# ansonb/FeTA_TMLR

Measured on AMD Instinct MI355X. Metric: graphs/sec fwd+bwd, ZINC batch (N<=37,d=64,K=16), higher is better.
Workload: dtype f32; 1 GPU; ZINC-shaped synthetic padded-graph batch, ChebConvDynamic block (attention + coefficient generator + spectral filter), fwd+bwd; graphs_per_gpu=128, global_batch=128, n_pad=37, d_model=64, heads=4, filter_order=4, k_eig=16, filter_mode=spectral, layers=3, norm=batch(per-rank stats), hip_graph=True, backward=single, two_phase=False, graph_collectives=False, ranks=1, parallelism=dp1

## Files before the change

### feta_tmlr_amd/csrc/block_bwd.hip

```cpp
#include <cstdlib>
#include <type_traits>

#include "feta_abi_common.h"
#include "feta_colsum.h"
#include "feta_ln.h"
#include "feta_lp.h"
#include "feta_rowops.h"

namespace feta {

typedef feta_attn_block_grad BwdArgs;

constexpr int kBbD = 64, kBbH = 4, kBbDH = 16;
constexpr int kBbP = kBbD + 4;
constexpr int kBbThreads = 512;
constexpr int kBbMaxGrid = 256;

template <class T>
__host__ __device__ inline int block_bwd_lds_bytes(int nt, bool gbn, bool gln = false, int heads = kBbH) {
  const int nr = 16 * nt, P = kBbD + Lp<T>::PAD;
  return (int)sizeof(T) * 7 * nr * P
         + 4 * (nr * (nr + 1)
                + heads * nr * 2 + nr
                + 8 * kBbD + 8 * 2 * 16
                + (gbn ? 5 * kBbD + reduce_scratch_floats(kBbD, 512) : 0)
                + (gln ? 8 * 2 * kBbD : 0));
}

#ifdef FETA_TIMING
__device__ unsigned long long feta_bbwd_stamps[4 * 8 * 8];
__device__ unsigned int feta_bbwd_launch;
#endif
#define BB_STAMP(i) FETA_RT_STAMP(feta_bbwd_stamps, feta_bbwd_launch, i)

__device__ __forceinline__ void acc_to(float* p, float v, bool first) {
  if (first) *p = v;
  else atomicAdd(p, v);
}

template <class T, int NT, bool SPLIT, bool LOOP, bool TWO>
__global__ __launch_bounds__(kBbThreads) void attn_block_bwd_kernel(BwdArgs a, ColsumPlan sums, int main_grid) {
  if ((int)blockIdx.x >= main_grid) {
    colsum_role<kBbThreads>(sums, (int)blockIdx.x - main_grid);
    return;
  }
  typedef Lp<T> L;
  typedef typename L::Op Op;
  typedef typename L::Vec Vec;
  constexpr int NS = TWO ? 2 : 1;
  constexpr int D = kBbD, DH = kBbDH, H = kBbH * NS, P = kBbD + L::PAD, NR = 16 * NT, PEP = NR + 1;
  constexpr int VEC = L::VEC, RV = D / VEC;
  const int tid = threadIdx.x, lane = tid & 63, wv = tid >> 6, lq = lane & 15, g = lane >> 4;
  const int hp = SPLIT ? ((int)blockIdx.x >= a.B ? 1 : 0) : 0;
  const int h = SPLIT ? 2 * hp + (wv & 1) : (wv & 3);
  const int role = SPLIT ? ((wv >> 1) & 1) : (wv >> 2);
  const int half = wv >> 2;
  const int ct = SPLIT ? 2 * hp + (wv & 1) : (wv & 3);
  const int ktile = wv & 3;
  auto mine_dc = [&](int rt) { return SPLIT ? rt == (wv >> 1) : (rt & 1) == (wv >> 2); };
  auto mine_dx = [&](int rt) { return (rt & 1) == (wv >> 2); };
  T* Qs = reinterpret_cast<T*>(lds_bytes());
  T* Ks = Qs + NR * P;
  T* Vs = Ks + NR * P;
  T* Ds = Vs + NR * P;
  T* Os = Ds + NR * P;
  T* Gt = Os + NR * P;
  T* X0 = Gt + NR * P;
  float* PE = reinterpret_cast<float*>(X0 + NR * P);
  float* ST = PE + NR * PEP;
  float* RS = ST + H * NR * 2;
  float* DBO = RS + NR;
  float* DBS = DBO + 8 * D;
  float* gv = DBS + 8 * 2 * 16;
  const T* gdy = reinterpret_cast<const T*>(a.dy);
  const T* gy1 = reinterpret_cast<const T*>(a.y1);
  const T* gqkv = reinterpret_cast<const T*>(a.qkv);
  const T* gout = reinterpret_cast<const T*>(a.out);
  const T* gd2 = reinterpret_cast<const T*>(a.dout2);
  const T* gpe = reinterpret_cast<const T*>(a.pe);
  const T* gx0 = reinterpret_cast<const T*>(a.x0);
  const bool gbn = a.bn1 != nullptr;
  const bool gln = a.ln1_gamma != nullptr, x0ln = a.x0_ln_gamma != nullptr;
  const bool has_y1 = a.y1 != nullptr;
  float* DGL = gv;
  const bool has_pe = a.pe != nullptr;
  const bool want_sums = a.sum_out != nullptr;
  const bool xbn = a.bn0 != nullptr;
  const bool d2_f32 = a.dout2 != nullptr && a.dout2_f32 != 0 && sizeof(T) != sizeof(float);
  BB_STAMP(0);

  if (gbn) {
    float* scr = gv + 5 * D;
    const int cpre = min(tid, D - 1);
    const float bn_scale = a.bn1[cpre], bn_mean = a.bn1[2 * D + cpre], bn_rstd = a.bn1[3 * D + cpre];
    if (a.g_sum != nullptr) {
      reduce_partials_t<kBbThreads, 16>(a.g_sum, a.Gs, D, scr + 2 * D, scr);
      for (int c = tid; c < D; c += kBbThreads) {
        gv[3 * D + c] = scr[c] / (float)a.M;
        gv[4 * D + c] = scr[D + c] / (float)a.M;
        if (blockIdx.x == 0) {
          if (a.dbeta != nullptr) a.dbeta[c] = scr[c];
          if (a.dgamma != nullptr) a.dgamma[c] = scr[D + c];
          if (a.fin_out != nullptr) {
            a.fin_out[c] = gv[3 * D + c];
            a.fin_out[D + c] = gv[4 * D + c];
          }
        }
      }
    }
    if (tid < D) {
      gv[tid] = bn_scale;
      gv[D + tid] = bn_mean;
      gv[2 * D + tid] = bn_rstd;
    }
    __syncthreads();
  }
  float sc0 = 1.0f, sh0 = 0.0f, mean0[4] = {0.f, 0.f, 0.f, 0.f}, rstd0[4] = {0.f, 0.f, 0.f, 0.f};
  if (xbn) {
    sc0 = a.bn0[16 * ktile + lq];
    sh0 = a.bn0[D + 16 * ktile + lq];
#pragma unroll
    for (int r = 0; r < 4; ++r) {
      mean0[r] = a.bn0[2 * D + 16 * ktile + 4 * g + r];
      rstd0[r] = a.bn0[3 * D + 16 * ktile + 4 * g + r];
    }
  }
  const int nm1 = a.N - 1;
  float sum1[4] = {0.f, 0.f, 0.f, 0.f}, sum2[4] = {0.f, 0.f, 0.f, 0.f};
  const int nwg = main_grid;
  int b = (int)blockIdx.x - hp * a.B;
  const int lane0 = lane;
  do {
    int lane_l = lane0;
    if (LOOP) FETA_OPAQUE_LANE(lane_l);
    const int lane = lane_l, tid = (wv << 6) | lane, lq = lane & 15, g = lane >> 4;
    const bool first = !LOOP || b < nwg;
    if (LOOP && !first) __syncthreads();
    const float* w_out_l = a.w_out;
    const float* w_in_l = a.w_in;
    if (LOOP) {
      FETA_OPAQUE_PTR(w_out_l);
      FETA_OPAQUE_PTR(w_in_l);
    }
    const feta_gcf w_out_p = (feta_gcf)w_out_l, w_in_p = (feta_gcf)w_in_l;
    const int n = a.n_real[b];
    BB_STAMP(1);
    auto grow = [&](int node) { return (int64_t)b * a.row_sb + (int64_t)min(node, nm1) * a.row_sn; };

    constexpr int RI = (NR * RV + kBbThreads - 1) / kBbThreads;
    Vec qv[RI], kv[RI], vv[RI], ov[RI], dyv[RI], y1v[RI], x0v[RI], d2v[RI];
    float rsn[RI];
#pragma unroll
    for (int i = 0; i < RI; ++i) {
      const int idx = min(tid + kBbThreads * i, NR * RV - 1), c4 = VEC * (idx % RV);
      const int64_t row = grow(idx / RV);
      qv[i] = L::ldv(gqkv + row * 3 * D + c4);
      kv[i] = L::ldv(gqkv + row * 3 * D + D + c4);
      vv[i] = L::ldv(gqkv + row * 3 * D + 2 * D + c4);
      ov[i] = L::ldv(gout + row * D + c4);
      dyv[i] = L::ldv(gdy + row * D + c4);
      y1v[i] = L::ldv((has_y1 ? gy1 : gdy) + row * D + c4);
      x0v[i] = L::ldv(gx0 + row * D + c4);
      if (d2_f32) {
        float f[VEC];
#pragma unroll
        for (int e = 0; e < VEC; e += 4) {
          const float4 t4 = *reinterpret_cast<const float4*>(a.dout2 + row * D + c4 + e);
          f[e] = t4.x; f[e + 1] = t4.y; f[e + 2] = t4.z; f[e + 3] = t4.w;
        }
        d2v[i] = L::pack(f);
      } else {
        d2v[i] = L::ldv((a.dout2 != nullptr ? gd2 : gdy) + row * D + c4);
      }
      rsn[i] = a.rowscale != nullptr ? a.rowscale[row] : 1.0f;
    }
    constexpr int PEI = (NR * NR + kBbThreads - 1) / kBbThreads;
    float pev[PEI];
#pragma unroll
    for (int i = 0; i < PEI; ++i) {
      const int idx = tid + kBbThreads * i, qq = idx / NR, kk = idx - qq * NR;
      const float v = has_pe ? L::ld1(gpe + ((int64_t)b * a.N + min(qq, nm1)) * a.N + min(kk, nm1)) : 1.0f;
      pev[i] = (idx < NR * NR && qq < a.N && kk < a.N) ? v : 0.0f;
    }
    {
      const int hh = tid / (NR * 2), rem = tid - hh * NR * 2;
      const float sv = a.attn_stats[(((int64_t)b * H + min(hh, H - 1)) * a.N + min(rem >> 1, nm1)) * 2 + (rem & 1)];
      if (tid < H * NR * 2) ST[tid] = sv;
      if constexpr (TWO) {
        const int idx = tid + kBbThreads, h2 = idx / (NR * 2), rem2 = idx - h2 * NR * 2;
        const float sv2 = a.attn_stats[(((int64_t)b * H + min(h2, H - 1)) * a.N + min(rem2 >> 1, nm1)) * 2 + (rem2 & 1)];
        if (idx < H * NR * 2) ST[idx] = sv2;
      }
      if (tid < NR) RS[tid] = (a.rowscale != nullptr && tid < a.N) ? a.rowscale[grow(tid)] : (tid < a.N ? 1.0f : 0.0f);
    }
    float dbo[VEC];
#pragma unroll
    for (int e = 0; e < VEC; ++e) dbo[e] = 0.0f;
    float gl1[VEC], gl0[VEC], bl0[VEC], dgam[VEC], dbet[VEC];
    {
      const float* p1 = gln ? a.ln1_gamma : a.w_out;
      const float* p0 = x0ln ? a.x0_ln_gamma : a.w_out;
      const float* q0 = x0ln ? a.x0_ln_beta : a.w_out;
      if (LOOP) {
        FETA_OPAQUE_PTR(p1);
        FETA_OPAQUE_PTR(p0);
        FETA_OPAQUE_PTR(q0);
      }
      const feta_gcf p1g = (feta_gcf)p1, p0g = (feta_gcf)p0, q0g = (feta_gcf)q0;
      const int c0v = VEC * (tid % RV);
#pragma unroll
      for (int e = 0; e < VEC; ++e) {
        gl1[e] = p1g[c0v + e];
        gl0[e] = p0g[c0v + e];
        bl0[e] = q0g[c0v + e];
        dgam[e] = dbet[e] = 0.0f;
      }
    }
#pragma unroll
    for (int i = 0; i < RI; ++i) {
      const int idx = tid + kBbThreads * i;
      if (idx < NR * RV) {
        const int node = idx / RV, c4 = VEC * (idx % RV), off = node * P + c4;
        const bool rk = node < a.N;
        const bool rkv = node < n;
        const bool dk2 = node < a.N && a.dout2 != nullptr;
        auto put = [&](T* dst, const Vec& v, bool keep) {
          float f[VEC];
          L::unpack(v, f);
#pragma unroll
          for (int e = 0; e < VEC; ++e) f[e] = keep ? f[e] : 0.0f;
          L::stv(dst + off, L::pack(f));
        };
        put(Qs, qv[i], rk);
        put(Ks, kv[i], rkv);
        put(Vs, vv[i], rkv);
        put(Os, ov[i], rk);
        if (x0ln) {
          float f[VEC];
          L::unpack(x0v[i], f);
          ln_apply<VEC>(f, gl0, bl0, a.ln_eps);
#pragma unroll
          for (int e = 0; e < VEC; ++e) f[e] = rk ? f[e] : 0.0f;
          L::stv(X0 + off, L::pack(f));
        } else {
          put(X0, x0v[i], rk);
        }
        put(Ds, d2v[i], dk2);
        float v[VEC];
        L::unpack(dyv[i], v);
        if (gln) {
          float yy[VEC];
          L::unpack(y1v[i], yy);
          ln_backward<VEC>(v, yy, gl1, a.ln_eps, rk, dgam, dbet);
        }
        if (gbn) {
          float yy[VEC];
          L::unpack(y1v[i], yy);
#pragma unroll
          for (int s = 0; s < VEC; ++s) {
            const int o = c4 + s;
            const float xh = (yy[s] - gv[D + o]) * gv[2 * D + o];
            v[s] = gv[o] * (v[s] - gv[3 * D + o] - xh * gv[4 * D + o]);
          }
        }
#pragma unroll
        for (int s = 0; s < VEC; ++s) {
          v[s] = rk ? v[s] : 0.0f;
          dbo[s] += rsn[i] * v[s];
        }
        L::stv(Gt + off, L::pack(v));
      }
    }
#pragma unroll
    for (int e = 0; e < VEC; ++e) {
      float sv = dbo[e];
      if (RV <= 8) sv += shfl_xor(sv, 8);
      sv += shfl_xor(sv, 16);
      sv += shfl_xor(sv, 32);
      if (lane < RV) DBO[wv * D + VEC * lane + e] = sv;
    }
    if (gln) {
#pragma unroll
      for (int e = 0; e < VEC; ++e) {
        float sg = dgam[e], sb = dbet[e];
        if (RV <= 8) {
          sg += shfl_xor(sg, 8);
          sb += shfl_xor(sb, 8);
        }
        sg += shfl_xor(sg, 16);
        sb += shfl_xor(sb, 16);
        sg += shfl_xor(sg, 32);
        sb += shfl_xor(sb, 32);
        if (lane < RV) {
          DGL[(wv * 2 + 0) * D + VEC * lane + e] = sg;
          DGL[(wv * 2 + 1) * D + VEC * lane + e] = sb;
        }
      }
    }
#pragma unroll
    for (int i = 0; i < PEI; ++i) {
      const int idx = tid + kBbThreads * i;
      if (idx < NR * NR) PE[(idx / NR) * PEP + idx % NR] = pev[i];
    }
    __syncthreads();
    BB_STAMP(2);
    float* prow = a.partial + (int64_t)(SPLIT ? b : (int)blockIdx.x) *
                                  (a.partial_ld > 0 ? (int64_t)a.partial_ld
                                                    : (int64_t)(4 * D * D + 4 * D + (gln ? 2 * D : 0)));
    if (hp == 0 && tid < D) {
      float sv = 0.0f;
#pragma unroll
      for (int w8 = 0; w8 < 8; ++w8) sv += DBO[w8 * D + tid];
      acc_to(prow + D * D + tid, sv, first);
    }
    if (gln && hp == 0 && tid >= D && tid < 3 * D) {
      const int which = (tid - D) / D, c = (tid - D) % D;
      float sv = 0.0f;
#pragma unroll
      for (int w8 = 0; w8 < 8; ++w8) sv += DGL[(w8 * 2 + which) * D + c];
      acc_to(prow + 4 * D * D + 4 * D + which * D + c, sv, first);
    }

    {
      Op woA[4];
#pragma unroll
      for (int j = 0; j < 4; ++j) {
        const feta_gcf p = w_out_p + (int64_t)(16 * j + 4 * g) * D + 16 * ct + lq;
        woA[j] = L::mk(p[0], p[D], p[2 * D], p[3 * D]);
      }
#pragma unroll
      for (int rt = 0; rt < NT; ++rt) {
        if (!mine_dc(rt)) continue;
        const int rowl = 16 * rt + lq;
        RowOp<T, D> gf;
        load_row_op_scaled<T, D>(gf, Gt + rowl * P, g, RS[rowl]);
        f32x4 acc = zero4();
#pragma unroll
        for (int j = 0; j < 4; ++j) acc = L::mma(woA[j], gf.o[j], acc);
        T* dst = Ds + rowl * P + 16 * ct + 4 * g;
        float d2[4];
        L::ld4(dst, d2);
        L::st4(dst, acc[0] + d2[0], acc[1] + d2[1], acc[2] + d2[2], acc[3] + d2[3]);
      }
    }
    __syncthreads();
    BB_STAMP(3);

    const int co = DH * h;
    f32x4 r0[NT], r1[NT];
#pragma unroll
    for (int t = 0; t < NT; ++t) {
      r0[t] = zero4();
      r1[t] = zero4();
    }
    if constexpr (!TWO) {
    if (role == 0) {
      Op kf[NT], vf[NT], kb[NT];
#pragma unroll
      for (int t = 0; t < NT; ++t) {
        const int rowl = 16 * t + lq;
        kf[t] = L::ld(Ks + rowl * P + co + 4 * g);
        vf[t] = L::ld(Vs + rowl * P + co + 4 * g);
        kb[t] = L::gather(Ks + (16 * t + 4 * g) * P + co + lq, P);
      }
#pragma unroll
      for (int qb = 0; qb < NT; ++qb) {
        const int q = 16 * qb + lq;
        const Op qf = L::ld_scaled(Qs + q * P + co + 4 * g, a.scale);
        const Op dof = L::ld(Ds + q * P + co + 4 * g);
        const Op of = L::ld(Os + q * P + co + 4 * g);
        float delta = L::get(dof, 0) * L::get(of, 0) + L::get(dof, 1) * L::get(of, 1) + L::get(dof, 2) * L::get(of, 2) +
                      L::get(dof, 3) * L::get(of, 3);
        delta += shfl_xor(delta, 16);
        delta += shfl_xor(delta, 32);
        const float m = ST[(h * NR + q) * 2], z = ST[(h * NR + q) * 2 + 1];
        const float rinv = fast_rcp(fmaxf(z, 1e-6f));
        if (z < 1e-6f) delta = 0.0f;
#pragma unroll
        for (int kt = 0; kt < NT; ++kt) {
          if (16 * kt >= n) continue;
          if (SPLIT && ((qb * NT + kt) & 1) != half) continue;
          const f32x4 s = L::mma(kf[kt], qf, zero4());
          const f32x4 da = L::mma(vf[kt], dof, zero4());
          float pd[4];
#pragma unroll
          for (int r = 0; r < 4; ++r) {
            const int key = 16 * kt + 4 * g + r;
            const float p = key < n ? fast_exp(s[r] - m) * PE[q * PEP + key] * rinv : 0.0f;
            pd[r] = p * (da[r] - delta);
          }
          r0[qb] = L::mma(L::mk(pd[0], pd[1], pd[2], pd[3]), kb[kt], r0[qb]);
        }
      }
    } else {
      Op qf[NT], dof[NT], qb4[NT], dob[NT];
      float sd[NT][4], mq[NT][4], rz[NT][4];
#pragma unroll
      for (int t = 0; t < NT; ++t) {
        const int rowl = 16 * t + lq;
        qf[t] = L::ld_scaled(Qs + rowl * P + co + 4 * g, a.scale);
        dof[t] = L::ld(Ds + rowl * P + co + 4 * g);
        const T* colq = Qs + (16 * t + 4 * g) * P + co + lq;
        const T* cold = Ds + (16 * t + 4 * g) * P + co + lq;
        const T* colo = Os + (16 * t + 4 * g) * P + co + lq;
        float qv4[4], dv4[4];
#pragma unroll
        for (int r = 0; r < 4; ++r) {
          const int rr = 16 * t + 4 * g + r;
          const bool ok = rr < a.N;
          dv4[r] = L::ld1(cold + r * P);
          qv4[r] = L::ld1(colq + r * P) * a.scale;
          sd[t][r] = row16_sum(dv4[r] * L::ld1(colo + r * P));
          const float z = ST[(h * NR + rr) * 2 + 1];
          mq[t][r] = ST[(h * NR + rr) * 2];
          rz[t][r] = ok ? fast_rcp(fmaxf(z, 1e-6f)) : 0.0f;
          if (z < 1e-6f) sd[t][r] = 0.0f;
        }
        qb4[t] = L::mk(qv4[0], qv4[1], qv4[2], qv4[3]);
        dob[t] = L::mk(dv4[0], dv4[1], dv4[2], dv4[3]);
      }
#pragma unroll
      for (int kt = 0; kt < NT; ++kt) {
        if (16 * kt >= n) continue;
        const int key = 16 * kt + lq;
        const Op kf = L::ld(Ks + key * P + co + 4 * g);
        const Op vf = L::ld(Vs + key * P + co + 4 * g);
#pragma unroll
        for (int qb = 0; qb < NT; ++qb) {
          if (SPLIT && ((kt * NT + qb) & 1) != half) continue;
          const f32x4 s = L::mma(qf[qb], kf, zero4());
          const f32x4 da = L::mma(dof[qb], vf, zero4());
          float pp[4], ds[4];
#pragma unroll
          for (int r = 0; r < 4; ++r) {
            const int q = 16 * qb + 4 * g + r;
            pp[r] = key < n ? fast_exp(s[r] - mq[qb][r]) * PE[q * PEP + key] * rz[qb][r] : 0.0f;
            ds[r] = pp[r] * (da[r] - sd[qb][r]);
          }
          r1[kt] = L::mma(L::mk(pp[0], pp[1], pp[2], pp[3]), dob[qb], r1[kt]);
          r0[kt] = L::mma(L::mk(ds[0], ds[1], ds[2], ds[3]), qb4[qb], r0[kt]);
        }
      }
    }
    } else {
    auto attn_head = [&](auto shc) __attribute__((always_inline)) {
    constexpr int sh = decltype(shc)::value;
    int lane_h = lane;
    if (LOOP) FETA_OPAQUE_LANE(lane_h);
    const int lq = lane_h & 15, g = lane_h >> 4;
    const bool ga = (g >> 1) == sh, la = (lq >> 3) == sh;
    const int hs = NS * h + sh;
    auto mg = [&](const Op& x) __attribute__((always_inline)) { return L::sel(ga, x, L::zero()); };
    auto ml = [&](const Op& x) __attribute__((always_inline)) { return L::sel(la, x, L::zero()); };
    if (role == 0) {
      Op kf[NT], vf[NT], kb[NT];
#pragma unroll
      for (int t = 0; t < NT; ++t) {
        const int rowl = 16 * t + lq;
        kf[t] = L::ld(Ks + rowl * P + co + 4 * g);
        vf[t] = L::ld(Vs + rowl * P + co + 4 * g);
        kb[t] = ml(L::gather(Ks + (16 * t + 4 * g) * P + co + lq, P));
      }
#pragma unroll
      for (int qb = 0; qb < NT; ++qb) {
        const int q = 16 * qb + lq;
        const Op qf = mg(L::ld_scaled(Qs + q * P + co + 4 * g, a.scale));
        const Op dof = mg(L::ld(Ds + q * P + co + 4 * g));
        const Op of = L::ld(Os + q * P + co + 4 * g);
        float delta = L::get(dof, 0) * L::get(of, 0) + L::get(dof, 1) * L::get(of, 1) + L::get(dof, 2) * L::get(of, 2) +
                      L::get(dof, 3) * L::get(of, 3);
        delta += shfl_xor(delta, 16);
        delta += shfl_xor(delta, 32);
        const float m = ST[(hs * NR + q) * 2], z = ST[(hs * NR + q) * 2 + 1];
        const float rinv = fast_rcp(fmaxf(z, 1e-6f));
        if (z < 1e-6f) delta = 0.0f;
#pragma unroll
        for (int kt = 0; kt < NT; ++kt) {
          if (16 * kt >= n) continue;
          if (SPLIT && ((qb * NT + kt) & 1) != half) continue;
          const f32x4 s = L::mma(kf[kt], qf, zero4());
          const f32x4 da = L::mma(vf[kt], dof, zero4());
          float pd[4];
#pragma unroll
          for (int r = 0; r < 4; ++r) {
            const int key = 16 * kt + 4 * g + r;
            const float p = key < n ? fast_exp(s[r] - m) * PE[q * PEP + key] * rinv : 0.0f;
            pd[r] = p * (da[r] - delta);
          }
          r0[qb] = L::mma(L::mk(pd[0], pd[1], pd[2], pd[3]), kb[kt], r0[qb]);
        }
      }
    } else {
      Op qf[NT], dof[NT], qb4[NT], dob[NT];
      float sd[NT][4], mq[NT][4], rz[NT][4];
#pragma unroll
      for (int t = 0; t < NT; ++t) {
        const int rowl = 16 * t + lq;
        qf[t] = mg(L::ld_scaled(Qs + rowl * P + co + 4 * g, a.scale));
        dof[t] = mg(L::ld(Ds + rowl * P + co + 4 * g));
        const T* colq = Qs + (16 * t + 4 * g) * P + co + lq;
        const T* cold = Ds + (16 * t + 4 * g) * P + co + lq;
        const T* colo = Os + (16 * t + 4 * g) * P + co + lq;
        float qv4[4], dv4[4];
#pragma unroll
        for (int r = 0; r < 4; ++r) {
          const int rr = 16 * t + 4 * g + r;
          const bool ok = rr < a.N;
          dv4[r] = L::ld1(cold + r * P);
          qv4[r] = L::ld1(colq + r * P) * a.scale;
          if (!la) dv4[r] = qv4[r] = 0.0f;
          sd[t][r] = row16_sum(dv4[r] * L::ld1(colo + r * P));
          const float z = ST[(hs * NR + rr) * 2 + 1];
          mq[t][r] = ST[(hs * NR + rr) * 2];
          rz[t][r] = ok ? fast_rcp(fmaxf(z, 1e-6f)) : 0.0f;
          if (z < 1e-6f) sd[t][r] = 0.0f;
        }
        qb4[t] = L::mk(qv4[0], qv4[1], qv4[2], qv4[3]);
        dob[t] = L::mk(dv4[0], dv4[1], dv4[2], dv4[3]);
      }
#pragma unroll
      for (int kt = 0; kt < NT; ++kt) {
        if (16 * kt >= n) continue;
        const int key = 16 * kt + lq;
        const Op kf = L::ld(Ks + key * P + co + 4 * g);
        const Op vf = L::ld(Vs + key * P + co + 4 * g);
#pragma unroll
        for (int qb = 0; qb < NT; ++qb) {
          if (SPLIT && ((kt * NT + qb) & 1) != half) continue;
          const Op qfq = LOOP ? mg(L::ld_scaled(Qs + (16 * qb + lq) * P + co + 4 * g, a.scale)) : qf[qb];
          const Op dfq = LOOP ? mg(L::ld(Ds + (16 * qb + lq) * P + co + 4 * g)) : dof[qb];
          const f32x4 s = L::mma(qfq, kf, zero4());
          const f32x4 da = L::mma(dfq, vf, zero4());
          float pp[4], ds[4];
#pragma unroll
          for (int r = 0; r < 4; ++r) {
            const int q = 16 * qb + 4 * g + r;
            pp[r] = key < n ? fast_exp(s[r] - mq[qb][r]) * PE[q * PEP + key] * rz[qb][r] : 0.0f;
            ds[r] = pp[r] * (da[r] - sd[qb][r]);
          }
          r1[kt] = L::mma(L::mk(pp[0], pp[1], pp[2], pp[3]), dob[qb], r1[kt]);
          r0[kt] = L::mma(L::mk(ds[0], ds[1], ds[2], ds[3]), qb4[qb], r0[kt]);
        }
      }
    }
    };
    attn_head(std::integral_constant<int, 0>{});
    attn_head(std::integral_constant<int, 1>{});
    }
    {
      float c0 = 0.0f, c1 = 0.0f;
#pragma unroll
      for (int t = 0; t < NT; ++t)
#pragma unroll
        for (int r = 0; r < 4; ++r) {
          c0 += r0[t][r];
          c1 += r1[t][r];
        }
      c0 += shfl_xor(c0, 16);
      c0 += shfl_xor(c0, 32);
      c1 += shfl_xor(c1, 16);
      c1 += shfl_xor(c1, 32);
      if (g == 0) {
        DBS[(wv * 2 + 0) * 16 + lq] = role == 0 ? c0 * a.scale : c0;
        DBS[(wv * 2 + 1) * 16 + lq] = c1;
      }
    }
    constexpr int NWO = SPLIT ? 2 : 4;
    if (role == 0) {
      const int ot = SPLIT ? (wv & 1) + 2 * (wv >> 2) : (wv & 3);
      f32x4 aWo[NWO];
#pragma unroll
      for (int i = 0; i < NWO; ++i) aWo[i] = zero4();
#pragma unroll 1
      for (int q4 = 0; q4 < NT; ++q4) {
        const int rr = 16 * q4 + g;
        float gvv[4];
#pragma unroll
        for (int s4 = 0; s4 < 4; ++s4) gvv[s4] = RS[rr + 4 * s4] * L::ld1(Gt + (rr + 4 * s4) * P + 16 * ot + lq);
        const Op ga = L::mk(gvv[0], gvv[1], gvv[2], gvv[3]);
#pragma unroll
        for (int i = 0; i < NWO; ++i)
          aWo[i] = L::mma(ga, L::gather(Os + rr * P + 16 * (SPLIT ? 2 * hp + i : i) + lq, 4 * P), aWo[i]);
      }
#pragma unroll
      for (int i = 0; i < NWO; ++i)
#pragma unroll
        for (int r = 0; r < 4; ++r)
        {
          acc_to(prow + (int64_t)(16 * ot + 4 * g + r) * D + 16 * (SPLIT ? 2 * hp + i : i) + lq, aWo[i][r], first);
        }
    }
    BB_STAMP(4);
    __syncthreads();
#pragma unroll
    for (int pass = 0; pass < (SPLIT ? 2 : 1); ++pass) {
      if (!SPLIT || half == pass) {
#pragma unroll
        for (int t = 0; t < NT; ++t) {
#pragma unroll
          for (int r = 0; r < 4; ++r) {
            const int rr = 16 * t + 4 * g + r;
            if (role == 0) {
              T* dq = Qs + rr * P + co + lq;
              L::st1(dq, (pass == 0 ? 0.0f : L::ld1(dq)) + r0[t][r] * a.scale);
            } else {
              T* dk = Ks + rr * P + co + lq;
              T* dv = Vs + rr * P + co + lq;
              L::st1(dk, (pass == 0 ? 0.0f : L::ld1(dk)) + r0[t][r]);
              L::st1(dv, (pass == 0 ? 0.0f : L::ld1(dv)) + r1[t][r]);
            }
          }
        }
      }
      __syncthreads();
    }

    BB_STAMP(5);
    constexpr int NJX = SPLIT ? 2 : 4;
    f32x4 dxa[NT];
#pragma unroll
    for (int rt = 0; rt < NT; ++rt) dxa[rt] = zero4();
#pragma unroll
    for (int part = 0; part < 3; ++part) {
      Op wiA[NJX];
#pragma unroll
      for (int j = 0; j < NJX; ++j) {
        const feta_gcf p = w_in_p + (int64_t)(64 * part + 16 * (SPLIT ? 2 * hp + j : j) + 4 * g) * D + 16 * ktile + lq;
        wiA[j] = L::mk(p[0], p[D], p[2 * D], p[3 * D]);
      }
#pragma unroll
      for (int rt = 0; rt < NT; ++rt) {
        if (!mine_dx(rt)) continue;
        const T* drow = (part == 0 ? Qs : (part == 1 ? Ks : Vs)) + (16 * rt + lq) * P + (SPLIT ? 32 * hp : 0);
#pragma unroll
        for (int j = 0; j < NJX; ++j) dxa[rt] = L::mma(wiA[j], L::ld(drow + 16 * j + 4 * g), dxa[rt]);
      }
    }
    T* dxo = reinterpret_cast<T*>((SPLIT && hp == 1) ? a.dx_b : a.dx);
    const float resw = (SPLIT && hp == 1) ? 0.0f : 1.0f;
#pragma unroll
    for (int rt = 0; rt < NT; ++rt) {
      if (!mine_dx(rt)) continue;
      const int rowl = 16 * rt + lq;
      const f32x4 acc = dxa[rt];
      float res[4];
      L::ld4(Gt + rowl * P + 16 * ktile + 4 * g, res);
      const float v[4] = {acc[0] + resw * res[0], acc[1] + resw * res[1], acc[2] + resw * res[2], acc[3] + resw * res[3]};
      const bool rok = rowl < a.N;
      if (rok) L::st4(dxo + grow(rowl) * D + 16 * ktile + 4 * g, v[0], v[1], v[2], v[3]);
      if (want_sums) {
        float xx[4];
        L::ld4(X0 + rowl * P + 16 * ktile + 4 * g, xx);
#pragma unroll
        for (int r = 0; r < 4; ++r) {
          const float s1 = rok ? v[r] : 0.0f;
          sum1[r] += s1;
          sum2[r] += s1 * (xx[r] - mean0[r]) * rstd0[r];
        }
      }
    }
    if (want_sums) {
      float s1v[4], s2v[4];
#pragma unroll
      for (int r = 0; r < 4; ++r) {
        s1v[r] = row16_sum(sum1[r]);
        s2v[r] = row16_sum(sum2[r]);
      }
      if (SPLIT) {
        float* red = PE;
        if ((wv >> 2) == 1 && lq == 0) {
#pragma unroll
          for (int r = 0; r < 4; ++r) {
            red[(ktile * 2 + 0) * 16 + 4 * g + r] = s1v[r];
            red[(ktile * 2 + 1) * 16 + 4 * g + r] = s2v[r];
          }
        }
        __syncthreads();
        if ((wv >> 2) == 0 && lq == 0) {
#pragma unroll
          for (int r = 0; r < 4; ++r) {
            a.sum_out[((int64_t)blockIdx.x * 2 + 0) * D + 16 * ktile + 4 * g + r] = s1v[r] + red[(ktile * 2 + 0) * 16 + 4 * g + r];
            a.sum_out[((int64_t)blockIdx.x * 2 + 1) * D + 16 * ktile + 4 * g + r] = s2v[r] + red[(ktile * 2 + 1) * 16 + 4 * g + r];
          }
        }
      } else if (lq == 0 && (!LOOP || b + nwg >= a.B)) {
        const int64_t prow2 = (int64_t)blockIdx.x * 2 + (wv >> 2);
#pragma unroll
        for (int r = 0; r < 4; ++r) {
          a.sum_out[(prow2 * 2 + 0) * D + 16 * ktile + 4 * g + r] = s1v[r];
          a.sum_out[(prow2 * 2 + 1) * D + 16 * ktile + 4 * g + r] = s2v[r];
        }
      }
    }

    BB_STAMP(6);
    constexpr int NWI = SPLIT ? 3 : 6;
    const int grp = wv >> 2;
    f32x4 aWi[NWI];
#pragma unroll
    for (int i = 0; i < NWI; ++i) aWi[i] = zero4();
    auto wi_part = [&](int i) { return SPLIT ? (3 * grp + i) >> 1 : (6 * grp + i) >> 2; };
    auto wi_head = [&](int i) { return SPLIT ? 2 * hp + ((3 * grp + i) & 1) : ((6 * grp + i) & 3); };
#pragma unroll 1
    for (int q4 = 0; q4 < NT; ++q4) {
      const int rr = 16 * q4 + g;
      float xv4[4];
#pragma unroll
      for (int s4 = 0; s4 < 4; ++s4) xv4[s4] = L::ld1(X0 + (rr + 4 * s4) * P + 16 * ktile + lq) * sc0 + sh0;
      const Op xb = L::mk(xv4[0], xv4[1], xv4[2], xv4[3]);
#pragma unroll
      for (int i = 0; i < NWI; ++i) {
        const int part = wi_part(i);
        const T* src = part == 0 ? Qs : (part == 1 ? Ks : Vs);
        aWi[i] = L::mma(L::gather(src + rr * P + 16 * wi_head(i) + lq, 4 * P), xb, aWi[i]);
      }
    }
    float* pWi = prow + D * D + D;
    float* pbi = pWi + 3 * D * D;
#pragma unroll
    for (int i = 0; i < NWI; ++i)
#pragma unroll
      for (int r = 0; r < 4; ++r)
      {
        acc_to(pWi + (int64_t)(64 * wi_part(i) + 16 * wi_head(i) + 4 * g + r) * D + 16 * ktile + lq, aWi[i][r], first);
      }
    if (tid < 3 * D) {
      const int part = tid >> 6, hh = (tid >> 4) & 3, c = tid & 15;
      const int rl = part == 0 ? 0 : 1, which = part == 2 ? 1 : 0;
      if (SPLIT) {
        if ((hh >> 1) == hp) {
          const int wa = (hh & 1) + 2 * rl;
          pbi[tid] = DBS[(wa * 2 + which) * 16 + c] + DBS[((wa + 4) * 2 + which) * 16 + c];
        }
      } else {
        acc_to(pbi + tid, DBS[((hh + 4 * rl) * 2 + which) * 16 + c], first);
      }
    }
    b += nwg;
  } while (LOOP && b < a.B);
  BB_STAMP(7);
  FETA_RT_LAUNCH_DONE(feta_bbwd_launch);
}

template <class T, int NT, bool TWO = false>
int launch_block_bwd(const BwdArgs& a, const feta_colsum_seg* segs, int nseg, hipStream_t stream) {
  size_t lds = block_bwd_lds_bytes<T>(NT, a.bn1 != nullptr, a.ln1_gamma != nullptr, TWO ? 2 * kBbH : kBbH);
  const int grid = feta_attn_block_bwd_blocks(a.B);
  ColsumPlan plan{};
  const int tiles = plan_colsum(segs, nseg, plan);
  if (tiles > 0 && lds < sizeof(float) * colsum_role_lds_floats(kBbThreads)) lds = sizeof(float) * colsum_role_lds_floats(kBbThreads);
  if (a.dx_b != nullptr) {
    auto kern = attn_block_bwd_kernel<T, NT, true, false, TWO>;
    static LdsSeen lds_seen;
    allow_dynamic_lds(kern, lds, lds_seen);
    hipLaunchKernelGGL(kern, dim3(2 * a.B + tiles), dim3(kBbThreads), lds, stream, a, plan, 2 * a.B);
  } else if (grid == a.B) {
    auto kern = attn_block_bwd_kernel<T, NT, false, false, TWO>;
    static LdsSeen lds_seen;
    allow_dynamic_lds(kern, lds, lds_seen);
    hipLaunchKernelGGL(kern, dim3(grid + tiles), dim3(kBbThreads), lds, stream, a, plan, grid);
  } else {
    auto kern = attn_block_bwd_kernel<T, NT, false, true, TWO>;
    static LdsSeen lds_seen;
    allow_dynamic_lds(kern, lds, lds_seen);
    hipLaunchKernelGGL(kern, dim3(grid + tiles), dim3(kBbThreads), lds, stream, a, plan, grid);
  }
  return check_launch("feta_attn_block_bwd");
}

template <class T>
int dispatch_block_bwd(const BwdArgs& a, const feta_colsum_seg* segs, int nseg, hipStream_t stream) {
  switch ((a.N + 15) / 16) {
    case 1: return launch_block_bwd<T, 1>(a, segs, nseg, stream);
    case 2: return launch_block_bwd<T, 2>(a, segs, nseg, stream);
    case 3: return launch_block_bwd<T, 3>(a, segs, nseg, stream);
    default: return launch_block_bwd<T, 4>(a, segs, nseg, stream);
  }
}

static int dispatch_block_bwd_two(const BwdArgs& a, const feta_colsum_seg* segs, int nseg, hipStream_t stream) {
  switch ((a.N + 15) / 16) {
    case 1: return launch_block_bwd<float, 1, true>(a, segs, nseg, stream);
    case 2: return launch_block_bwd<float, 2, true>(a, segs, nseg, stream);
    case 3: return launch_block_bwd<float, 3, true>(a, segs, nseg, stream);
    default: return launch_block_bwd<float, 4, true>(a, segs, nseg, stream);
  }
}

}

using namespace feta;

#ifdef FETA_TIMING
extern "C" int feta_debug_bbwd_stamps(unsigned long long* out256) {
  return (int)hipMemcpyFromSymbol(out256, HIP_SYMBOL(feta_bbwd_stamps), sizeof(unsigned long long) * 256);
}
#endif

extern "C" int feta_attn_block_bwd_supported(int N, int d_model, int heads) {
  return (d_model == kBbD && (heads == 4 || heads == 8) && N >= 1 && N <= 64) ? 1 : 0;
}

extern "C" int feta_attn_block_bwd_blocks(int B) {
  int cap = kBbMaxGrid;
  if (const char* e = getenv("FETA_BLOCK_BWD_MAX_GRID")) cap = atoi(e) > 0 ? atoi(e) : cap;
  return B < 1 ? 0 : (B < cap ? B : cap);
}

extern "C" int feta_attn_block_bwd(const feta_attn_block_grad* d, feta_stream_t stream) {
  return feta_attn_block_bwd_sums(d, nullptr, 0, stream);
}

extern "C" int feta_attn_block_bwd_sums(const feta_attn_block_grad* d, const feta_colsum_seg* segs, int nseg,
                                        feta_stream_t stream) {
  FETA_REQUIRE(d != nullptr, "attn_block_bwd: null descriptor");
  FETA_REQUIRE(nseg >= 0 && nseg <= FETA_COLSUM_MAX_SEGS && (nseg == 0 || segs != nullptr),
               "attn_block_bwd: 0..%d column-sum segments", FETA_COLSUM_MAX_SEGS);
  for (int i = 0; i < nseg; ++i) FETA_REQUIRE(colsum_seg_ok(segs[i]), "attn_block_bwd: bad segment %d", i);
  const BwdArgs& a = *d;
  FETA_REQUIRE(a.dy && a.w_out && a.w_in && a.qkv && a.out && a.n_real && a.attn_stats && a.x0 && a.dx && a.partial,
               "attn_block_bwd: null pointer");
  FETA_REQUIRE(a.B > 0, "attn_block_bwd: B=%d", a.B);
  FETA_REQUIRE(a.dx_b == nullptr || feta_attn_block_bwd_blocks(a.B) == a.B,
               "attn_block_bwd: the two-workgroup form (dx_b) needs one workgroup per graph (B=%d > %d)", a.B,
               feta_attn_block_bwd_blocks(a.B));
  FETA_REQUIRE(a.N >= 1 && a.N <= 64 && a.M == a.B * a.N, "attn_block_bwd: N=%d outside [1,64] or M != B*N", a.N);
  FETA_REQUIRE(!a.y1 || a.ln1_gamma || (a.bn1 && a.g_sum && a.Gs > 0), "attn_block_bwd: y1 needs bn1, g_sum, Gs - or ln1_gamma");
  FETA_REQUIRE(!a.bn1 || a.y1, "attn_block_bwd: bn1 needs y1");
  FETA_REQUIRE(!a.ln1_gamma || (a.y1 && !a.bn1 && !a.g_sum), "attn_block_bwd: ln1_gamma needs y1 and excludes bn1 / g_sum");
  FETA_REQUIRE(!a.x0_ln_gamma || (a.x0_ln_beta && !a.bn0 && !a.sum_out), "attn_block_bwd: x0_ln_gamma needs x0_ln_beta and excludes bn0 / sum_out");
  FETA_REQUIRE(!a.sum_out || a.bn0, "attn_block_bwd: sum_out needs bn0");
  FETA_REQUIRE(aligned16(a.dy) && aligned16(a.qkv) && aligned16(a.out) && aligned16(a.x0) && aligned16(a.dx) &&
               aligned16(a.y1) && aligned16(a.dout2) && aligned16(a.g_sum) && aligned16(a.dx_b),
               "attn_block_bwd: tensors must be 16-byte aligned");
  FETA_REQUIRE(a.dtype == FETA_F32 || a.dtype == FETA_BF16, "attn_block_bwd: dtype %d", a.dtype);
  FETA_REQUIRE(a.H == 0 || a.H == 4 || a.H == 8, "attn_block_bwd: H=%d (0 = 4, 4 or 8 heads)", a.H);
  if (a.H == 8) {
    FETA_REQUIRE(a.dtype == FETA_F32, "attn_block_bwd: 8 heads need fp32 storage");
    return dispatch_block_bwd_two(a, segs, nseg, (hipStream_t)stream);
  }
  if (a.dtype == FETA_BF16) return dispatch_block_bwd<bf16_t>(a, segs, nseg, (hipStream_t)stream);
  return dispatch_block_bwd<float>(a, segs, nseg, (hipStream_t)stream);
}
```

### feta_tmlr_amd/csrc/feta_lp.h

```cpp
#pragma once
#include "feta_tiles.h"

namespace feta {

template <class T>
struct Lp;

template <>
struct Lp<float> {
  static constexpr int VEC = 4;
  static constexpr int PAD = 4;
  struct Op {
    float v[4];
  };
  struct Vec {
    float4 raw;
  };
  static __device__ __forceinline__ Op zero() { return Op{{0.0f, 0.0f, 0.0f, 0.0f}}; }
  static __device__ __forceinline__ Op mk(float a, float b, float c, float d) { return Op{{a, b, c, d}}; }
  static __device__ __forceinline__ Op mk(const f32x4& a) { return Op{{a[0], a[1], a[2], a[3]}}; }
  static __device__ __forceinline__ Op ld(const float* p) {
    const float4 x = *reinterpret_cast<const float4*>(p);
    return Op{{x.x, x.y, x.z, x.w}};
  }
  static __device__ __forceinline__ Op ldo(const Op* p) { return ld(reinterpret_cast<const float*>(p)); }
  static __device__ __forceinline__ void sto(Op* p, const Op& o) {
    *reinterpret_cast<float4*>(p) = make_float4(o.v[0], o.v[1], o.v[2], o.v[3]);
  }
  static __device__ __forceinline__ Op ld_scaled(const float* p, float s) {
    const float4 x = *reinterpret_cast<const float4*>(p);
    return Op{{x.x * s, x.y * s, x.z * s, x.w * s}};
  }
  static __device__ __forceinline__ Op gather(const float* p, int stride) {
    return Op{{p[0], p[stride], p[2 * stride], p[3 * stride]}};
  }
  static __device__ __forceinline__ float get(const Op& o, int i) { return o.v[i]; }
  static __device__ __forceinline__ Op sel(bool c, const Op& a, const Op& b) {
    return Op{{c ? a.v[0] : b.v[0], c ? a.v[1] : b.v[1], c ? a.v[2] : b.v[2], c ? a.v[3] : b.v[3]}};
  }
  static __device__ __forceinline__ f32x4 mma(const Op& a, const Op& b, f32x4 acc) {
#pragma unroll
    for (int s = 0; s < 4; ++s) acc = mfma16(a.v[s], b.v[s], acc);
    return acc;
  }
  static __device__ __forceinline__ float ld1(const float* p) { return *p; }
  static __device__ __forceinline__ float to_f(float v) { return v; }
  static __device__ __forceinline__ float one() { return 1.0f; }
  static __device__ __forceinline__ void st1(float* p, float v) { *p = v; }
  static __device__ __forceinline__ void ld4(const float* p, float (&v)[4]) {
    const float4 x = *reinterpret_cast<const float4*>(p);
    v[0] = x.x; v[1] = x.y; v[2] = x.z; v[3] = x.w;
  }
  static __device__ __forceinline__ void st4(float* p, float a, float b, float c, float d) {
    *reinterpret_cast<float4*>(p) = make_float4(a, b, c, d);
  }
  static __device__ __forceinline__ Vec ldv(const float* p) { return Vec{*reinterpret_cast<const float4*>(p)}; }
  static __device__ __forceinline__ void stv(float* p, const Vec& v) { *reinterpret_cast<float4*>(p) = v.raw; }
  static __device__ __forceinline__ void unpack(const Vec& v, float (&f)[VEC]) {
    f[0] = v.raw.x; f[1] = v.raw.y; f[2] = v.raw.z; f[3] = v.raw.w;
  }
  static __device__ __forceinline__ Vec pack(const float (&f)[VEC]) { return Vec{make_float4(f[0], f[1], f[2], f[3])}; }
};

template <>
struct Lp<bf16_t> {
  static constexpr int VEC = 8;
  static constexpr int PAD = 8;
  typedef bf16x4_pk Op;
  struct __attribute__((aligned(16))) Vec {
    bf16x4_pk lo, hi;
  };
  static __device__ __forceinline__ Op zero() { return pack_bf16x4(0.0f, 0.0f, 0.0f, 0.0f); }
  static __device__ __forceinline__ Op mk(float a, float b, float c, float d) { return pack_bf16x4(a, b, c, d); }
  static __device__ __forceinline__ Op mk(const f32x4& a) { return pack_bf16x4(a[0], a[1], a[2], a[3]); }
  static __device__ __forceinline__ Op ld(const bf16_t* p) { return *reinterpret_cast<const bf16x4_pk*>(p); }
  static __device__ __forceinline__ Op ldo(const Op* p) { return *p; }
  static __device__ __forceinline__ void sto(Op* p, const Op& o) { *p = o; }
  static __device__ __forceinline__ Op ld_scaled(const bf16_t* p, float s) {
    const Op x = ld(p);
    return pack_bf16x4(bf16x4_get(x, 0) * s, bf16x4_get(x, 1) * s, bf16x4_get(x, 2) * s, bf16x4_get(x, 3) * s);
  }
  static __device__ __forceinline__ Op gather(const bf16_t* p, int stride) {
    return pack_bf16x4_raw(p[0], p[stride], p[2 * stride], p[3 * stride]);
  }
  static __device__ __forceinline__ float get(const Op& o, int i) { return bf16x4_get(o, i); }
  static __device__ __forceinline__ Op sel(bool c, const Op& a, const Op& b) {
    Op r;
    r.v[0] = c ? a.v[0] : b.v[0]; r.v[1] = c ? a.v[1] : b.v[1]; r.v[2] = c ? a.v[2] : b.v[2]; r.v[3] = c ? a.v[3] : b.v[3];
    return r;
  }
  static __device__ __forceinline__ f32x4 mma(const Op& a, const Op& b, f32x4 acc) { return mfma16_bf16_pk(a, b, acc); }
  static __device__ __forceinline__ float ld1(const bf16_t* p) { return bf2f(*p); }
  static __device__ __forceinline__ float to_f(bf16_t v) { return bf2f(v); }
  static __device__ __forceinline__ bf16_t one() { return f2bf(1.0f); }
  static __device__ __forceinline__ void st1(bf16_t* p, float v) { *p = f2bf(v); }
  static __device__ __forceinline__ void ld4(const bf16_t* p, float (&v)[4]) {
    const Op x = ld(p);
    v[0] = bf16x4_get(x, 0); v[1] = bf16x4_get(x, 1); v[2] = bf16x4_get(x, 2); v[3] = bf16x4_get(x, 3);
  }
  static __device__ __forceinline__ void st4(bf16_t* p, float a, float b, float c, float d) {
    *reinterpret_cast<bf16x4_pk*>(p) = pack_bf16x4(a, b, c, d);
  }
  static __device__ __forceinline__ Vec ldv(const bf16_t* p) { return *reinterpret_cast<const Vec*>(p); }
  static __device__ __forceinline__ void stv(bf16_t* p, const Vec& v) { *reinterpret_cast<Vec*>(p) = v; }
  static __device__ __forceinline__ void unpack(const Vec& v, float (&f)[VEC]) {
#pragma unroll
    for (int i = 0; i < 4; ++i) {
      f[i] = bf16x4_get(v.lo, i);
      f[4 + i] = bf16x4_get(v.hi, i);
    }
  }
  static __device__ __forceinline__ Vec pack(const float (&f)[VEC]) {
    Vec v;
    v.lo = pack_bf16x4(f[0], f[1], f[2], f[3]);
    v.hi = pack_bf16x4(f[4], f[5], f[6], f[7]);
    return v;
  }
};

template <class T, int DH>
struct RowOp {
  static constexpr int NJ = (DH + 15) / 16;
  typename Lp<T>::Op o[NJ];
};

template <class T, int DH>
__device__ __forceinline__ void load_row_op(RowOp<T, DH>& t, const T* row, int g) {
#pragma unroll
  for (int j = 0; j < RowOp<T, DH>::NJ; ++j) t.o[j] = Lp<T>::ld(row + 16 * j + 4 * g);
}
template <class T, int DH>
__device__ __forceinline__ void load_row_op_scaled(RowOp<T, DH>& t, const T* row, int g, float scale) {
#pragma unroll
  for (int j = 0; j < RowOp<T, DH>::NJ; ++j) t.o[j] = Lp<T>::ld_scaled(row + 16 * j + 4 * g, scale);
}
template <class T, int DH>
__device__ __forceinline__ f32x4 dot_row_ops(const RowOp<T, DH>& a, const RowOp<T, DH>& b, f32x4 acc) {
#pragma unroll
  for (int j = 0; j < RowOp<T, DH>::NJ; ++j) acc = Lp<T>::mma(a.o[j], b.o[j], acc);
  return acc;
}

__device__ __forceinline__ char* lds_bytes() { return reinterpret_cast<char*>(feta_lds); }

}
```

Before: 496,200 graphs/s.

## Stage transposed w_out/w_in weights in LDS and use LDS-only barriers in block backward

Before, each wave gathered w_out and w_in from global memory with strided scalar loads. Now the attention-block backward kernel prefetches those weights into registers early, commits them transposed into extra LDS, and reads MFMA operands with vector LDS loads. When LDS budget allows only part of w_in, the remaining parts are preloaded into registers early. It also swaps __syncthreads for an LDS-only barrier, which is selected by default. In exchange the kernel uses more LDS and registers, which may lower occupancy, and global loads are no longer fenced at those barriers.

Measured after the change: 494,400 graphs/s. No clear change (-0.4%).

```diff
diff --git a/feta_tmlr_amd/csrc/block_bwd.hip b/feta_tmlr_amd/csrc/block_bwd.hip
--- a/feta_tmlr_amd/csrc/block_bwd.hip
+++ b/feta_tmlr_amd/csrc/block_bwd.hip
@@ -27,6 +27,16 @@
                 + (gln ? 8 * 2 * kBbD : 0));
 }
 
+constexpr int kBbLdsLimit = 160 * 1024;
+constexpr int kBbWoP = kBbD + 4;
+__host__ __device__ constexpr int block_bwd_wc(bool split) { return split ? 32 : 64; }
+__host__ __device__ constexpr int block_bwd_wout_floats(bool split) { return block_bwd_wc(split) * kBbWoP; }
+__host__ __device__ constexpr int block_bwd_win_part_floats(bool split) { return kBbD * (block_bwd_wc(split) + 4); }
+template <class T>
+__host__ __device__ inline int block_bwd_wbase_bytes(int nt, bool gbn, bool gln, int heads) {
+  return (block_bwd_lds_bytes<T>(nt, gbn, gln, heads) + 15) & ~15;
+}
+
 #ifdef FETA_TIMING
 __device__ unsigned long long feta_bbwd_stamps[4 * 8 * 8];
 __device__ unsigned int feta_bbwd_launch;
@@ -39,7 +49,7 @@
 }
 
 template <class T, int NT, bool SPLIT, bool LOOP, bool TWO>
-__global__ __launch_bounds__(kBbThreads) void attn_block_bwd_kernel(BwdArgs a, ColsumPlan sums, int main_grid) {
+__global__ __launch_bounds__(kBbThreads) void attn_block_bwd_kernel(BwdArgs a, ColsumPlan sums, int main_grid, int wst) {
   if ((int)blockIdx.x >= main_grid) {
     colsum_role<kBbThreads>(sums, (int)blockIdx.x - main_grid);
     return;
@@ -87,7 +97,54 @@
   const bool want_sums = a.sum_out != nullptr;
   const bool xbn = a.bn0 != nullptr;
   const bool d2_f32 = a.dout2 != nullptr && a.dout2_f32 != 0 && sizeof(T) != sizeof(float);
+  const bool lds_only = (wst & 8) != 0;
+  auto barrier = [&]() __attribute__((always_inline)) {
+    if (lds_only) lds_barrier();
+    else __syncthreads();
+  };
+  constexpr bool CANW = std::is_same<T, float>::value && NT <= 3;
+  constexpr int WC = block_bwd_wc(SPLIT), WIP = WC + 4, WOP = kBbWoP;
+  constexpr int UW = WC / 32;
+  const bool st_o = CANW && (wst & 1) != 0;
+  const int st_i = CANW ? (wst >> 1) & 3 : 0;
+  float* WoT = reinterpret_cast<float*>(lds_bytes() + block_bwd_wbase_bytes<T>(NT, gbn, gln, H));
+  float* WiT = WoT + block_bwd_wout_floats(SPLIT);
+  float4 wreg[4 * UW];
+  auto stage_request = [&]() __attribute__((always_inline)) {
+    if constexpr (CANW) {
+      const int l15 = lane & 15, c4 = 4 * (lane >> 4), c0 = SPLIT ? 32 * hp : 0;
+#pragma unroll
+      for (int i = 0; i < UW; ++i) {
+        const int u = wv + 8 * i;
+        if (st_o) wreg[i] = *reinterpret_cast<const float4*>(a.w_out + (16 * (u / (WC / 16)) + l15) * D + c0 + 16 * (u % (WC / 16)) + c4);
+#pragma unroll
+        for (int p = 0; p < 3; ++p)
+          if (p < st_i) wreg[UW * (1 + p) + i] = *reinterpret_cast<const float4*>(a.w_in + (64 * p + c0 + 16 * (u >> 2) + l15) * D + 16 * (u & 3) + c4);
+      }
+    }
+  };
+  auto stage_commit = [&]() __attribute__((always_inline)) {
+    if constexpr (CANW) {
+      const int l15 = lane & 15, c4 = 4 * (lane >> 4);
+#pragma unroll
+      for (int i = 0; i < UW; ++i) {
+        const int u = wv + 8 * i;
+        if (st_o) {
+          float* dst = WoT + (16 * (u % (WC / 16)) + c4) * WOP + 16 * (u / (WC / 16)) + l15;
+          dst[0] = wreg[i].x; dst[WOP] = wreg[i].y; dst[2 * WOP] = wreg[i].z; dst[3 * WOP] = wreg[i].w;
+        }
+#pragma unroll
+        for (int p = 0; p < 3; ++p)
+          if (p < st_i) {
+            const float4 w = wreg[UW * (1 + p) + i];
+            float* dst = WiT + p * block_bwd_win_part_floats(SPLIT) + (16 * (u & 3) + c4) * WIP + 16 * (u >> 2) + l15;
+            dst[0] = w.x; dst[WIP] = w.y; dst[2 * WIP] = w.z; dst[3 * WIP] = w.w;
+          }
+      }
+    }
+  };
   BB_STAMP(0);
+  stage_request();
 
   if (gbn) {
     float* scr = gv + 5 * D;
@@ -113,8 +170,9 @@
       gv[D + tid] = bn_mean;
       gv[2 * D + tid] = bn_rstd;
     }
-    __syncthreads();
+    barrier();
   }
+  if (LOOP) stage_commit();
   float sc0 = 1.0f, sh0 = 0.0f, mean0[4] = {0.f, 0.f, 0.f, 0.f}, rstd0[4] = {0.f, 0.f, 0.f, 0.f};
   if (xbn) {
     sc0 = a.bn0[16 * ktile + lq];
@@ -135,7 +193,7 @@
     if (LOOP) FETA_OPAQUE_LANE(lane_l);
     const int lane = lane_l, tid = (wv << 6) | lane, lq = lane & 15, g = lane >> 4;
     const bool first = !LOOP || b < nwg;
-    if (LOOP && !first) __syncthreads();
+    if (LOOP && !first) barrier();
     const float* w_out_l = a.w_out;
     const float* w_in_l = a.w_in;
     if (LOOP) {
@@ -182,6 +240,7 @@
       const float v = has_pe ? L::ld1(gpe + ((int64_t)b * a.N + min(qq, nm1)) * a.N + min(kk, nm1)) : 1.0f;
       pev[i] = (idx < NR * NR && qq < a.N && kk < a.N) ? v : 0.0f;
     }
+    if (!LOOP) stage_commit();
     {
       const int hh = tid / (NR * 2), rem = tid - hh * NR * 2;
       const float sv = a.attn_stats[(((int64_t)b * H + min(hh, H - 1)) * a.N + min(rem >> 1, nm1)) * 2 + (rem & 1)];
@@ -302,7 +361,7 @@
       const int idx = tid + kBbThreads * i;
       if (idx < NR * NR) PE[(idx / NR) * PEP + idx % NR] = pev[i];
     }
-    __syncthreads();
+    barrier();
     BB_STAMP(2);
     float* prow = a.partial + (int64_t)(SPLIT ? b : (int)blockIdx.x) *
                                   (a.partial_ld > 0 ? (int64_t)a.partial_ld
@@ -323,10 +382,16 @@
 
     {
       Op woA[4];
-#pragma unroll
-      for (int j = 0; j < 4; ++j) {
-        const feta_gcf p = w_out_p + (int64_t)(16 * j + 4 * g) * D + 16 * ct + lq;
-        woA[j] = L::mk(p[0], p[D], p[2 * D], p[3 * D]);
+      if (st_o) {
+        const float* p = WoT + (16 * (SPLIT ? (wv & 1) : ct) + lq) * WOP + 4 * g;
+#pragma unroll
+        for (int j = 0; j < 4; ++j) woA[j] = L::ldw(p + 16 * j);
+      } else {
+#pragma unroll
+        for (int j = 0; j < 4; ++j) {
+          const feta_gcf p = w_out_p + (int64_t)(16 * j + 4 * g) * D + 16 * ct + lq;
+          woA[j] = L::mk(p[0], p[D], p[2 * D], p[3 * D]);
+        }
       }
 #pragma unroll
       for (int rt = 0; rt < NT; ++rt) {
@@ -343,7 +408,7 @@
         L::st4(dst, acc[0] + d2[0], acc[1] + d2[1], acc[2] + d2[2], acc[3] + d2[3]);
       }
     }
-    __syncthreads();
+    barrier();
     BB_STAMP(3);
 
     const int co = DH * h;
@@ -590,8 +655,22 @@
           acc_to(prow + (int64_t)(16 * ot + 4 * g + r) * D + 16 * (SPLIT ? 2 * hp + i : i) + lq, aWo[i][r], first);
         }
     }
+    constexpr int NJX = SPLIT ? 2 : 4;
+    Op wiE[3][NJX];
+    const bool early = !LOOP && st_o;
+    if (early) {
+#pragma unroll
+      for (int part = 0; part < 3; ++part)
+        if (part >= st_i) {
+#pragma unroll
+          for (int j = 0; j < NJX; ++j) {
+            const feta_gcf p = w_in_p + (int64_t)(64 * part + 16 * (SPLIT ? 2 * hp + j : j) + 4 * g) * D + 16 * ktile + lq;
+            wiE[part][j] = L::mk(p[0], p[D], p[2 * D], p[3 * D]);
+          }
+        }
+    }
     BB_STAMP(4);
-    __syncthreads();
+    barrier();
 #pragma unroll
     for (int pass = 0; pass < (SPLIT ? 2 : 1); ++pass) {
       if (!SPLIT || half == pass) {
@@ -612,21 +691,29 @@
           }
         }
       }
-      __syncthreads();
+      barrier();
     }
 
     BB_STAMP(5);
-    constexpr int NJX = SPLIT ? 2 : 4;
     f32x4 dxa[NT];
 #pragma unroll
     for (int rt = 0; rt < NT; ++rt) dxa[rt] = zero4();
 #pragma unroll
     for (int part = 0; part < 3; ++part) {
       Op wiA[NJX];
-#pragma unroll
-      for (int j = 0; j < NJX; ++j) {
-        const feta_gcf p = w_in_p + (int64_t)(64 * part + 16 * (SPLIT ? 2 * hp + j : j) + 4 * g) * D + 16 * ktile + lq;
-        wiA[j] = L::mk(p[0], p[D], p[2 * D], p[3 * D]);
+      if (part < st_i) {
+        const float* p = WiT + part * block_bwd_win_part_floats(SPLIT) + (16 * ktile + lq) * WIP + 4 * g;
+#pragma unroll
+        for (int j = 0; j < NJX; ++j) wiA[j] = L::ldw(p + 16 * j);
+      } else if (early) {
+#pragma unroll
+        for (int j = 0; j < NJX; ++j) wiA[j] = wiE[part][j];
+      } else {
+#pragma unroll
+        for (int j = 0; j < NJX; ++j) {
+          const feta_gcf p = w_in_p + (int64_t)(64 * part + 16 * (SPLIT ? 2 * hp + j : j) + 4 * g) * D + 16 * ktile + lq;
+          wiA[j] = L::mk(p[0], p[D], p[2 * D], p[3 * D]);
+        }
       }
 #pragma unroll
       for (int rt = 0; rt < NT; ++rt) {
@@ -675,7 +762,7 @@
             red[(ktile * 2 + 1) * 16 + 4 * g + r] = s2v[r];
           }
         }
-        __syncthreads();
+        barrier();
         if ((wv >> 2) == 0 && lq == 0) {
 #pragma unroll
           for (int r = 0; r < 4; ++r) {
@@ -742,9 +829,28 @@
   FETA_RT_LAUNCH_DONE(feta_bbwd_launch);
 }
 
+template <class T, int NT>
+static int block_bwd_wstage(const BwdArgs& a, bool split, int heads, size_t& lds) {
+  const char* e = getenv("FETA_BLOCK_BWD_LDS_W");
+  if (e != nullptr && e[0] == '0') return 0;
+  int wst = 8;
+  if (!std::is_same<T, float>::value || NT > 3 || !aligned16(a.w_out) || !aligned16(a.w_in)) return wst;
+  const int base = block_bwd_wbase_bytes<T>(NT, a.bn1 != nullptr, a.ln1_gamma != nullptr, heads);
+  const int wo = 4 * block_bwd_wout_floats(split), wi = 4 * block_bwd_win_part_floats(split);
+  const int main_wgs = split ? 2 * a.B : feta_attn_block_bwd_blocks(a.B);
+  const int per_cu = (main_wgs > kBbMaxGrid && 2 * base <= kBbLdsLimit) ? 2 : 1;
+  const int budget = kBbLdsLimit / per_cu;
+  if (base + wo > budget) return wst;
+  int parts = (budget - base - wo) / wi;
+  parts = parts < 3 ? parts : 3;
+  lds = (size_t)(base + wo + parts * wi);
+  return wst | 1 | (parts << 1);
+}
+
 template <class T, int NT, bool TWO = false>
 int launch_block_bwd(const BwdArgs& a, const feta_colsum_seg* segs, int nseg, hipStream_t stream) {
   size_t lds = block_bwd_lds_bytes<T>(NT, a.bn1 != nullptr, a.ln1_gamma != nullptr, TWO ? 2 * kBbH : kBbH);
+  const int wst = block_bwd_wstage<T, NT>(a, a.dx_b != nullptr, TWO ? 2 * kBbH : kBbH, lds);
   const int grid = feta_attn_block_bwd_blocks(a.B);
   ColsumPlan plan{};
   const int tiles = plan_colsum(segs, nseg, plan);
@@ -753,17 +859,17 @@
     auto kern = attn_block_bwd_kernel<T, NT, true, false, TWO>;
     static LdsSeen lds_seen;
     allow_dynamic_lds(kern, lds, lds_seen);
-    hipLaunchKernelGGL(kern, dim3(2 * a.B + tiles), dim3(kBbThreads), lds, stream, a, plan, 2 * a.B);
+    hipLaunchKernelGGL(kern, dim3(2 * a.B + tiles), dim3(kBbThreads), lds, stream, a, plan, 2 * a.B, wst);
   } else if (grid == a.B) {
     auto kern = attn_block_bwd_kernel<T, NT, false, false, TWO>;
     static LdsSeen lds_seen;
     allow_dynamic_lds(kern, lds, lds_seen);
-    hipLaunchKernelGGL(kern, dim3(grid + tiles), dim3(kBbThreads), lds, stream, a, plan, grid);
+    hipLaunchKernelGGL(kern, dim3(grid + tiles), dim3(kBbThreads), lds, stream, a, plan, grid, wst);
   } else {
     auto kern = attn_block_bwd_kernel<T, NT, false, true, TWO>;
     static LdsSeen lds_seen;
     allow_dynamic_lds(kern, lds, lds_seen);
-    hipLaunchKernelGGL(kern, dim3(grid + tiles), dim3(kBbThreads), lds, stream, a, plan, grid);
+    hipLaunchKernelGGL(kern, dim3(grid + tiles), dim3(kBbThreads), lds, stream, a, plan, grid, wst);
   }
   return check_launch("feta_attn_block_bwd");
 }
diff --git a/feta_tmlr_amd/csrc/feta_lp.h b/feta_tmlr_amd/csrc/feta_lp.h
--- a/feta_tmlr_amd/csrc/feta_lp.h
+++ b/feta_tmlr_amd/csrc/feta_lp.h
@@ -27,6 +27,7 @@
   static __device__ __forceinline__ void sto(Op* p, const Op& o) {
     *reinterpret_cast<float4*>(p) = make_float4(o.v[0], o.v[1], o.v[2], o.v[3]);
   }
+  static __device__ __forceinline__ Op ldw(const float* p) { return ld(p); }
   static __device__ __forceinline__ Op ld_scaled(const float* p, float s) {
     const float4 x = *reinterpret_cast<const float4*>(p);
     return Op{{x.x * s, x.y * s, x.z * s, x.w * s}};
@@ -75,6 +76,10 @@
   static __device__ __forceinline__ Op mk(const f32x4& a) { return pack_bf16x4(a[0], a[1], a[2], a[3]); }
   static __device__ __forceinline__ Op ld(const bf16_t* p) { return *reinterpret_cast<const bf16x4_pk*>(p); }
   static __device__ __forceinline__ Op ldo(const Op* p) { return *p; }
+  static __device__ __forceinline__ Op ldw(const float* p) {
+    const float4 x = *reinterpret_cast<const float4*>(p);
+    return pack_bf16x4(x.x, x.y, x.z, x.w);
+  }
   static __device__ __forceinline__ void sto(Op* p, const Op& o) { *p = o; }
   static __device__ __forceinline__ Op ld_scaled(const bf16_t* p, float s) {
     const Op x = ld(p);
```
